# alipbcs/ZetaRay

Hardware: NVIDIA H100
Metric: Mpaths/s (1spp ReSTIR PT, 1080p) (higher is better)
Workload: dtype f32

## Files before the change

zetaray_b200/csrc/rdi.cu:

```cuda
#include "zr_pixel.cuh"
#include "zr_planes.h"
#include "zr_schedule.h"

#include "zr_rdi.cuh"

namespace zr
{
namespace
{
#ifndef ZR_RDI_TEMPORAL_THREADS
#define ZR_RDI_TEMPORAL_THREADS 768
#endif
#ifndef ZR_RDI_SPATIAL_THREADS
#define ZR_RDI_SPATIAL_THREADS 512
#endif
    static_assert(ZR_RDI_TEMPORAL_THREADS % 64 == 0 && ZR_RDI_SPATIAL_THREADS % 64 == 0, "a DI block is whole 8x8 groups");
    struct DiTemporalParked
    {
        Reservoir r;
        uint32_t pad[2];
    };
    static_assert(sizeof(DiTemporalParked) % 16 == 8, "DiTemporalParked must be 2 mod 4 words");
    constexpr size_t DI_TEMPORAL_SMEM_BYTES = (size_t)ZR_RDI_TEMPORAL_THREADS * sizeof(DiTemporalParked);

    template<uint32_t MF>
    __global__ void ZR_LB(ZR_RDI_TEMPORAL_THREADS) k_di_temporal(SceneDev sc, FrameView f, DIParams prm, zr_rdi_reservoir* __restrict__ resCurr,
        const zr_rdi_reservoir* __restrict__ resPrev, uint2* __restrict__ target, float4* __restrict__ finalImg, uint32_t dispX, uint32_t dispY,
        const uint32_t* __restrict__ order)
    {
        using SD = BSDF::ShadingDataT<MF>;
        extern __shared__ DiTemporalParked s_diTemporalParked[];
        const zr_frame_constants& fc = f.fc;
        uint2 sg = make_uint2(0, 0);
        const uint32_t groupFlat = order[blockIdx.x] * (ZR_RDI_TEMPORAL_THREADS / 64) + (threadIdx.x >> 6);
        const uint32_t tInGroup = threadIdx.x & 63;
        uint2 px = make_uint2(0xffffffffu, 0xffffffffu);
        if (groupFlat < dispX * dispY)
            px = SwizzleThreadGroup(groupFlat, 0, tInGroup & 7, tInGroup >> 3, 8, 8, dispX, 16, 4, 16 * dispY, sg);
        const long long t0 = clock64();
        bool act = !(px.x >= f.W || px.y >= f.H || px.y < prm.rowBegin || px.y >= prm.rowEnd);
        const uint32_t x = px.x, y = px.y;
        const size_t idx = act ? (size_t)y * f.W + x : 0;
        if (act)
        {
            const GFlags flags = FlagsAt(f.core, f.W, x, y);
            if (flags.invalid)
            {
                finalImg[idx] = f4(0, 0, 0, 0);
                act = false;
            }
            else if (flags.emissive && !prm.spatial)
            {
                WriteEmissive(fc, f, finalImg, idx);
                act = false;
            }
        }
        PixelT<SD> p;
        p.surface = SD::InitEmpty();
        p.pos = f3(0); p.normal = f3(0); p.roughness = 0;
        RNG rng_thread; rng_thread.State = 0;
        int numBsdfSamples = 0;
        if (act)
        {
            p = LoadPixel<SD>(f, sc, f.core, f.coat, x, y, false, x, y);
            rng_thread = RNG::Init(x, y, fc.FrameNum);
            numBsdfSamples = (!p.surface.GlossSpecular() && p.roughness < 0.3f) ? 2 : 1;
        }
        RNG rng_group = RNG::Init(groupFlat % dispX, groupFlat / dispX, fc.FrameNum);
        const uint32_t sampleSetIdx = rng_group.UniformUintBounded_Faster(sc.numSampleSets);
        Reservoir& r = s_diTemporalParked[threadIdx.x].r;
        RIS_InitialCandidates_Sync(r, act, sc, p.pos, p.normal, p.roughness, p.surface, sampleSetIdx, numBsdfSamples, rng_thread);
        if (prm.temporal)
        {
            float2 motionVec = f2(0, 0);
            TemporalCandidateT<SD> tc; tc.valid = false; tc.px = tc.py = 0; tc.pos = tc.normal = f3(0);
            tc.surface = SD::InitEmpty();
            ZR_PHASE();
            if (act)
            {
                motionVec = unpack_snorm16x2(__ldg(&f.me[idx].x));
                const float2 currUV = f2((float)x + 0.5f, (float)y + 0.5f) / f2((float)f.W, (float)f.H);
                const float2 prevUV = currUV - motionVec;
                tc = FindTemporalCandidate(f, sc, p.pos, p.normal, p.roughness, p.surface, prevUV);
            }
            TemporalResample1_Sync(act && tc.valid, sc, p.pos, p.normal, p.surface, tc, resPrev, f.W, r, rng_thread);
            if (act && prm.spatial)
            {
                const bool disoccluded = !tc.valid && (dot(motionVec, motionVec) > 0);
                r.target = disoccluded ? -r.target : r.target;
                WriteTarget(target, idx, r.target);
                r.target = Math::Sanitize(r.target);
            }
        }
        AccountCost(prm.costMap, f.W, f.H, px.x, px.y, t0);
        if (!act)
            return;
        if (prm.temporal || prm.reset)
        {
            zr_rdi_reservoir rec;
            r.Write(rec, prm.M_max);
            StoreRdi(&resCurr[idx], rec);
        }
        if (!prm.spatial || !prm.temporal)
            WriteFinal(fc, finalImg, idx, r.target * r.W);
    }

    template<uint32_t MF>
    __global__ void ZR_LB(ZR_RDI_SPATIAL_THREADS) k_di_spatial(SceneDev sc, FrameView f, DIParams prm, const zr_rdi_reservoir* __restrict__ resCurr,
        const uint2* __restrict__ target, float4* __restrict__ finalImg, uint32_t dispX, uint32_t dispY,
        const uint32_t* __restrict__ order)
    {
        using SD = BSDF::ShadingDataT<MF>;
        const zr_frame_constants& fc = f.fc;
        uint2 sg = make_uint2(0, 0);
        const uint32_t groupFlat = order[blockIdx.x] * (ZR_RDI_SPATIAL_THREADS / 64) + (threadIdx.x >> 6);
        const uint32_t tInGroup = threadIdx.x & 63;
        uint2 px = make_uint2(0xffffffffu, 0xffffffffu);
        if (groupFlat < dispX * dispY)
            px = SwizzleThreadGroup(groupFlat, 0, tInGroup & 7, tInGroup >> 3, 8, 8, dispX, 16, 4, 16 * dispY, sg);
        const long long t0 = clock64();
        bool active = px.x < f.W && px.y < f.H && px.y >= prm.rowBegin && px.y < prm.rowEnd;
        const int x = (int)px.x, y = (int)px.y;
        const size_t idx = active ? (size_t)y * f.W + x : 0;
        if (active)
        {
            const GFlags flags = FlagsAt(f.core, f.W, x, y);
            if (flags.invalid) active = false;
            else if (flags.emissive)
            {
                WriteEmissive(fc, f, finalImg, idx);
                active = false;
            }
        }
        PixelT<SD> p;
        p.surface = SD::InitEmpty();
        p.pos = f3(0); p.normal = f3(0); p.roughness = 0; p.z = 0;
        Reservoir r = Reservoir::Init();
        bool disoccluded = false;
        if (active)
        {
            p = LoadPixel<SD>(f, sc, f.core, f.coat, x, y, false, x, y);
            zr_rdi_reservoir rec;
            LoadRdi(&resCurr[idx], rec);
            r = Reservoir::Load(rec);
            if (r.lightIdx != UINT32_MAX_)
            {
                const zr_emissive_tri& tri = sc.emissives[r.lightIdx];
                r.lightID = tri.ID;
                const float3 vtx0 = Light::Vtx0(tri);
                const float3 vtx1 = Light::DecodeEmissiveTriV1(tri);
                const float3 vtx2 = Light::DecodeEmissiveTriV2(tri);
                r.lightPos = (1.0f - r.bary.x - r.bary.y) * vtx0 + r.bary.x * vtx1 + r.bary.y * vtx2;
                r.lightNormal = cross(vtx1 - vtx0, vtx2 - vtx0);
                r.lightNormal = dot(r.lightNormal, r.lightNormal) == 0 ? r.lightNormal : normalize(r.lightNormal);
                r.doubleSided = Light::IsDoubleSided(tri);
                r.target = LoadTarget(target, idx);
                disoccluded = r.target.x < 0 || r.target.y < 0 || r.target.z < 0;
                r.target = abs3(r.target);
            }
        }
        const uint32_t waveDisoccluded = __popc(__ballot_sync(0xffffffffu, active && disoccluded));
        RNG rng_group = RNG::Init(groupFlat % dispX, groupFlat / dispX, fc.FrameNum);
        rng_group.UniformUintBounded_Faster(sc.numSampleSets);
        const bool extra = !prm.stochasticSpatial || (rng_group.Uniform() < 0.6f);
        if (prm.extraDisocclusion)
            disoccluded = disoccluded && (waveDisoccluded > 3);
        int numSamples = extra ? 2 : 1;
        numSamples = !disoccluded ? numSamples : 4;
        RNG rng = RNG::Init((uint32_t)x, (uint32_t)y, fc.FrameNum);
        const float u0 = rng.Uniform();
        const int offset = (int)rng.UniformUintBounded_Faster(8);
        const float theta = u0 * TWO_PI;
        float sinTheta, cosTheta;
        zr_sincosf(theta, &sinTheta, &cosTheta);
        PairwiseMIS pairwiseMIS = PairwiseMIS::Init((uint32_t)numSamples, r);
        float3 samplePos[4]; int spx[4], spy[4]; uint32_t k = 0;
        ZR_PHASE();
        for (int i = 0; i < 4; i++)
        {
            if (!(active && i < numSamples)) continue;
            const float2 sampleUV = f2(c_disk32[((offset + i) & 31) * 2], c_disk32[((offset + i) & 31) * 2 + 1]);
            float2 rotated;
            rotated.x = dot(sampleUV, f2(cosTheta, -sinTheta));
            rotated.y = dot(sampleUV, f2(sinTheta, cosTheta));
            rotated = rotated * 16.0f;
            const float fx = fmaxf(rintf((float)x + rotated.x), 0.0f), fy = fmaxf(rintf((float)y + rotated.y), 0.0f);
            if (fx >= (float)f.W || fy >= (float)f.H) continue;
            const int qx = (int)fx, qy = (int)fy;
            float rough_i;
            const GFlags flags_i = FlagsAt(f.core, f.W, qx, qy, &rough_i);
            if (flags_i.invalid || flags_i.emissive) continue;
            const PixelT<SD> pi = LoadPixel<SD>(f, sc, f.core, f.coat, qx, qy, false, qx, qy);
            bool valid = PlaneHeuristicDI(pi.pos, p.normal, p.pos, p.z);
            valid = valid && (fabsf(rough_i - p.roughness) < 0.15f);
            if (!valid) continue;
            samplePos[k] = pi.pos; spx[k] = qx; spy[k] = qy;
            k++;
        }
        pairwiseMIS.k = k;
        for (uint32_t i = 0; i < 4; i++)
        {
            const bool go = active && (i < k);
            if (!__syncthreads_or(go))
                break;
            PixelT<SD> pi;
            pi.normal = f3(0);
            SD surface_i = SD::InitEmpty();
            Reservoir r_spatial = Reservoir::Init();
            float3 pos_i = f3(0);
            if (go)
            {
                pi = LoadPixel<SD>(f, sc, f.core, f.coat, spx[i], spy[i], false, spx[i], spy[i]);
                const uint4 c = ld128(&f.core[(size_t)spy[i] * f.W + spx[i]]);
                const float3 bc = f3((float)(c.z & 0xff) / 255.0f, (float)((c.z >> 8) & 0xff) / 255.0f, (float)((c.z >> 16) & 0xff) / 255.0f);
                const float bw = pi.flags.subsurface ? (float)(c.z >> 24) / 255.0f : 0.0f;
                pos_i = samplePos[i];
                const float3 wo_i = normalize(pi.origin - pos_i);
                surface_i = SD::Init(pi.normal, wo_i, pi.flags.metallic, pi.roughness, bc, BSDF::ETA_AIR,
                    pi.eta_next, pi.flags.transmissive, 0.0f, to_half(bw), pi.surface.coat_weight, pi.surface.coat_color,
                    pi.coatRoughness, pi.coatIor, sc.rho);
                zr_rdi_reservoir recN;
                LoadRdi(&resCurr[(size_t)spy[i] * f.W + spx[i]], recN);
                r_spatial = Reservoir::Load(recN);
            }
            pairwiseMIS.Stream_Sync(go, sc, r, p.pos, p.normal, p.surface, r_spatial, pos_i, pi.normal, surface_i, rng);
        }
        AccountCost(prm.costMap, f.W, f.H, px.x, px.y, t0);
        if (!active)
            return;
        pairwiseMIS.End(r, rng);
        const Reservoir rs = pairwiseMIS.r_s;
        WriteFinal(fc, finalImg, idx, rs.target * rs.W);
    }
}
}

struct zr_direct_pass
{
    uint32_t width = 0, height = 0;
    struct Sized
    {
        zr::Planes planes{ "zr_direct_pass" };
        zr_rdi_reservoir* d_res[2] = { nullptr, nullptr };
        uint2* d_target = nullptr;
        float4* d_final = nullptr;
    } sz;
    int currTemporalIdx = 0;
    bool isTemporalReservoirValid = false;
    bool resetTemporalTextures = true;
    bool patternLoaded = false;
    zr_direct_params params = Defaults();
    zr::LightingStrip strip{ "zr_direct_pass" };

    static zr_direct_params Defaults()
    {
        zr_direct_params p{};
        p.temporal_resample = 1; p.spatial_resample = 1; p.stochastic_spatial = 1; p.extra_disocclusion_sampling = 1;
        p.M_max = 20; p.alpha_min = 0.05f * 0.05f;
        return p;
    }
    zr_status Setup()
    {
        using zr::BSDF::MF_NONE; using zr::BSDF::MF_ALL;
        ZR_TRY(zr::ReserveParkedSmem(zr::k_di_temporal<MF_NONE>, ZR_RDI_TEMPORAL_THREADS, zr::DI_TEMPORAL_SMEM_BYTES, "zr_direct_pass: k_di_temporal"));
        ZR_TRY(zr::ReserveParkedSmem(zr::k_di_temporal<MF_ALL>, ZR_RDI_TEMPORAL_THREADS, zr::DI_TEMPORAL_SMEM_BYTES, "zr_direct_pass: k_di_temporal"));
        return ZR_OK;
    }
    zr_status OnWindowResized(uint32_t w, uint32_t h)
    {
        const size_t n = (size_t)w * h;
        Sized next;
        for (int i = 0; i < 2; i++) ZR_TRY(next.planes.Alloc(next.d_res[i], n));
        ZR_TRY(next.planes.Alloc(next.d_target, n));
        ZR_TRY(next.planes.Alloc(next.d_final, n));
        ZR_TRY(next.planes.Clear());
        sz = std::move(next);
        width = w; height = h;
        strip.ForgetSize();
        ResetFlags();
        return ZR_OK;
    }
    void ResetFlags() { currTemporalIdx = 0; isTemporalReservoirValid = false; resetTemporalTextures = true; }
    zr_status ResetTemporal()
    {
        ZR_TRY(sz.planes.Clear());
        ResetFlags();
        return ZR_OK;
    }
    zr_status LoadPattern()
    {
        if (patternLoaded) return ZR_OK;
        float pat[64];
        zr_status st = zr::read_asset("zr_direct_pass", "disk32.bin", pat, sizeof(pat));
        if (st != ZR_OK) return st;
        ZR_CUDA(cudaMemcpyToSymbol(zr::c_disk32, pat, 256));
        patternLoaded = true;
        return ZR_OK;
    }
    zr_status Render(const zr_frame_inputs* in, cudaStream_t stream)
    {
        using namespace zr;
        FrameView f;
        zr_status st = LightingFrame("zr_direct_pass", in, width, height, f);
        if (st != ZR_OK) return st;
        st = LoadPattern();
        if (st != ZR_OK) return st;
        const bool doTemporal = isTemporalReservoirValid && params.temporal_resample;
        const bool doSpatial = doTemporal && params.spatial_resample;
        if (doTemporal && (!in->prev.d_core || !in->prev.d_coat))
        {
            set_error("zr_direct_pass_render: temporal reuse needs the previous G-buffer");
            return ZR_ERR_INVALID_ARG;
        }
        DIParams prm{ doTemporal, doSpatial, params.stochastic_spatial, params.extra_disocclusion_sampling, params.M_max,
            params.alpha_min, resetTemporalTextures, strip.rowBegin, strip.ClampedRowEnd(height), strip.d_costMap };
        const uint32_t dispX = (width + 7) / 8, dispY = (height + 7) / 8;
        const int cur = currTemporalIdx;
        st = strip.Schedule(width, height, 8, 8, ZR_RDI_TEMPORAL_THREADS / 64, 0);
        if (st != ZR_OK) return st;
        st = strip.Schedule(width, height, 8, 8, ZR_RDI_SPATIAL_THREADS / 64, 1);
        if (st != ZR_OK) return st;
        const BlockSchedule& schedT = strip.sched[0];
        const BlockSchedule& schedS = strip.sched[1];
        const bool plain = (in->scene->materialFeatures & BSDF::MF_ALL) == 0;
        ZR_PROF("k_di_temporal", stream);
        (plain ? k_di_temporal<BSDF::MF_NONE> : k_di_temporal<BSDF::MF_ALL>)<<<schedT.count, ZR_RDI_TEMPORAL_THREADS, DI_TEMPORAL_SMEM_BYTES, stream>>>(in->scene->dev, f, prm, sz.d_res[cur], sz.d_res[1 - cur], sz.d_target, sz.d_final, dispX, dispY, schedT.d_order);
        ZR_LAUNCH_CHECK();
        strip.Exchange(sz.d_res[cur], width, height, 32u, stream);
        if (doSpatial)
        {
            ZR_PROF("k_di_spatial", stream);
            (plain ? k_di_spatial<BSDF::MF_NONE> : k_di_spatial<BSDF::MF_ALL>)<<<schedS.count, ZR_RDI_SPATIAL_THREADS, 0, stream>>>(in->scene->dev, f, prm, sz.d_res[cur], sz.d_target, sz.d_final, dispX, dispY, schedS.d_order);
            ZR_LAUNCH_CHECK();
        }
        isTemporalReservoirValid = true;
        currTemporalIdx = 1 - cur;
        resetTemporalTextures = false;
        return ZR_OK;
    }
};

extern "C"
{
    zr_status zr_direct_pass_create(uint32_t width, uint32_t height, zr_direct_pass** out) { return zr::CreatePass("zr_direct_pass", width, height, out); }
    zr_status zr_direct_pass_resize(zr_direct_pass* p, uint32_t width, uint32_t height) { return zr::ResizePass("zr_direct_pass", p, width, height); }
    zr_status zr_direct_pass_reset_temporal(zr_direct_pass* p) { return zr::ResetPass(p); }
    zr_status zr_direct_pass_default_params(zr_direct_params* out) { return zr::DefaultParams<zr_direct_pass>(out); }
    zr_status zr_direct_pass_set_params(zr_direct_pass* p, const zr_direct_params* params)
    {
        if (!p || !params) return ZR_ERR_INVALID_ARG;
        if (params->M_max == 0 || params->M_max > 31) { zr::set_error("zr_direct_pass_set_params: M_max must be in 1..31 (5-bit field)"); return ZR_ERR_INVALID_ARG; }
        p->params = *params;
        return ZR_OK;
    }
    zr_status zr_direct_pass_render(zr_direct_pass* p, const zr_frame_inputs* in, void* stream)
    {
        if (!p) return ZR_ERR_INVALID_ARG;
        return p->Render(in, (cudaStream_t)stream);
    }
    zr_status zr_direct_pass_set_rows(zr_direct_pass* p, uint32_t y0, uint32_t y1) { return p ? p->strip.SetRows(y0, y1, p->height) : ZR_ERR_INVALID_ARG; }
    zr_status zr_direct_pass_set_halo_exchange(zr_direct_pass* p, zr_halo_exchange_fn fn, void* user) { return p ? p->strip.SetHaloExchange(fn, user) : ZR_ERR_INVALID_ARG; }
    zr_status zr_direct_pass_set_schedule_costs(zr_direct_pass* p, const double* h_tile_cost, uint32_t tiles_x, uint32_t tiles_y)
    {
        return p ? p->strip.SetScheduleCosts(h_tile_cost, tiles_x, tiles_y, p->width, p->height) : ZR_ERR_INVALID_ARG;
    }
    zr_status zr_direct_pass_set_cost_map(zr_direct_pass* p, void* d_cycles) { return p ? p->strip.SetCostMap(d_cycles) : ZR_ERR_INVALID_ARG; }
    zr_status zr_direct_pass_get_output(zr_direct_pass* p, zr_direct_output id, zr_image2d* out)
    {
        if (!p || !out) return ZR_ERR_INVALID_ARG;
        const uint32_t w = p->width, h = p->height;
        switch (id)
        {
        case ZR_DIRECT_FINAL: *out = zr_image2d{ p->sz.d_final, w, h, w * 16u, 16u }; break;
        case ZR_DIRECT_RESERVOIR_CURR: *out = zr_image2d{ p->sz.d_res[1 - p->currTemporalIdx], w, h, w * 32u, 32u }; break;
        case ZR_DIRECT_TARGET: *out = zr_image2d{ p->sz.d_target, w, h, w * 8u, 8u }; break;
        default: zr::set_error("zr_direct_pass_get_output: unknown output id"); return ZR_ERR_INVALID_ARG;
        }
        return ZR_OK;
    }
    zr_status zr_direct_pass_describe_io(zr_direct_pass* p, zr_resource_use* uses, int* n)
    {
        if (!p || !uses || !n) return ZR_ERR_INVALID_ARG;
        uses[0] = zr_resource_use{ ZR_RES_GBUFFER_CURR, 0 };
        uses[1] = zr_resource_use{ ZR_RES_GBUFFER_PREV, 0 };
        uses[2] = zr_resource_use{ ZR_RES_SCENE_BVH, 0 };
        uses[3] = zr_resource_use{ ZR_RES_ALIAS_TABLE, 0 };
        uses[4] = zr_resource_use{ ZR_RES_DI_FINAL, 1 };
        *n = 5;
        return ZR_OK;
    }
    void zr_direct_pass_destroy(zr_direct_pass* p) { delete p; }
}
```

zetaray_b200/csrc/renderer.cu:

```cuda
#include <cuda_runtime.h>
#include <vector>
#include "../../include/zr_abi.h"
#include "zr_common.cuh"

struct zr_renderer
{
    uint32_t width = 0, height = 0;
    zr_scene* scene = nullptr;
    zr_gbuffer gbuffer[2]{};
    int curr = 0;
    uint64_t framesRendered = 0;
    zr_gbuffer_pass* gbufferPass = nullptr;
    zr_direct_pass* direct = nullptr;
    zr_indirect_pass* indirect = nullptr;
    zr_gi_pass* gi = nullptr;
    zr_integrator integrator = ZR_INTEGRATOR_RESTIR_PT;
    zr_compositing_pass* compositing = nullptr;
    zr_taa_pass* taa = nullptr;
    zr_svgf_pass* svgf = nullptr;
    zr_auto_exposure_pass* ae = nullptr;
    zr_display_pass* display = nullptr;
    cudaStream_t side = nullptr;
    cudaEvent_t evGBuffer = nullptr, evDirect = nullptr;
    bool twoStreams = true;
    zr_comm* comm = nullptr;
    int rank = 0, world = 1;
    std::vector<uint32_t> bounds;
    bool gatherOutput = true;
    static constexpr uint32_t HALO = 32;
    struct HookCtx { zr_renderer* r; int whichComm; } hookMain{ this, 0 }, hookSide{ this, 1 };
    zr_status hookStatus = ZR_OK;
    static void HaloHook(void* user, const zr_image2d* planes, int n, void* stream)
    {
        HookCtx* h = (HookCtx*)user;
        zr_renderer* r = h->r;
        const int which = (r->twoStreams && stream == (void*)r->side) ? 1 : 0;
        const zr_status s = zr_comm_exchange_halos(r->comm, which, r->bounds.data(), HALO, planes, n, stream);
        if (s != ZR_OK) r->hookStatus = s;
    }
    static void ReduceHook(void* user, uint32_t* d_values, uint32_t n, void* stream)
    {
        zr_renderer* r = (zr_renderer*)user;
        const zr_status s = zr_comm_allreduce_u32(r->comm, 0, d_values, n, stream);
        if (s != ZR_OK) r->hookStatus = s;
    }

    zr_status ApplyShard()
    {
        const bool sharded = comm && world > 1;
        const uint32_t y0 = sharded ? bounds[rank] : 0, y1 = sharded ? bounds[rank + 1] : height;
        zr_halo_exchange_fn hook = sharded ? HaloHook : nullptr;
        zr_status s = zr_gbuffer_pass_set_rows(gbufferPass, y0 > HALO ? y0 - HALO : 0, y1 + HALO < height ? y1 + HALO : height);
        if (s == ZR_OK) s = zr_direct_pass_set_rows(direct, y0, y1);
        if (s == ZR_OK) s = zr_indirect_pass_set_rows(indirect, y0, y1);
        if (s == ZR_OK) s = zr_compositing_pass_set_rows(compositing, y0 > 0 ? y0 - 1 : 0, y1 + 1 < height ? y1 + 1 : height);
        if (s == ZR_OK) s = zr_taa_pass_set_rows(taa, y0, y1);
        if (s == ZR_OK) s = zr_direct_pass_set_halo_exchange(direct, hook, &hookSide);
        if (s == ZR_OK) s = zr_indirect_pass_set_halo_exchange(indirect, hook, &hookMain);
        if (s == ZR_OK && gi) s = zr_gi_pass_set_rows(gi, y0, y1);
        if (s == ZR_OK && gi) s = zr_gi_pass_set_halo_exchange(gi, hook, &hookMain);
        if (s == ZR_OK && svgf) s = zr_svgf_pass_set_rows(svgf, y0, y1);
        if (s == ZR_OK && svgf) s = zr_svgf_pass_set_halo_exchange(svgf, hook, &hookMain);
        if (s == ZR_OK && ae) s = zr_auto_exposure_pass_set_rows(ae, y0, y1);
        if (s == ZR_OK && ae) s = zr_auto_exposure_pass_set_reduce(ae, sharded ? ReduceHook : nullptr, this);
        if (s == ZR_OK && display) s = zr_display_pass_set_rows(display, y0, y1);
        return s;
    }
    zr_status TakeHookStatus()
    {
        const zr_status s = hookStatus;
        hookStatus = ZR_OK;
        return s;
    }
    void ReleaseDisplay()
    {
        if (ae) zr_auto_exposure_pass_destroy(ae);
        if (display) zr_display_pass_destroy(display);
        ae = nullptr; display = nullptr;
    }

    void Release()
    {
        if (gbufferPass) zr_gbuffer_pass_destroy(gbufferPass);
        if (direct) zr_direct_pass_destroy(direct);
        if (indirect) zr_indirect_pass_destroy(indirect);
        if (gi) zr_gi_pass_destroy(gi);
        gi = nullptr;
        if (compositing) zr_compositing_pass_destroy(compositing);
        if (taa) zr_taa_pass_destroy(taa);
        if (svgf) zr_svgf_pass_destroy(svgf);
        svgf = nullptr;
        ReleaseDisplay();
        gbufferPass = nullptr; direct = nullptr; indirect = nullptr; compositing = nullptr; taa = nullptr;
        for (int i = 0; i < 2; i++) zr_gbuffer_free(&gbuffer[i]);
        if (side) cudaStreamDestroy(side);
        if (evGBuffer) cudaEventDestroy(evGBuffer);
        if (evDirect) cudaEventDestroy(evDirect);
        side = nullptr; evGBuffer = evDirect = nullptr;
    }
};

extern "C"
{
    zr_status zr_renderer_create(const zr_renderer_desc* desc, zr_scene* scene, zr_renderer** out)
    {
        if (!desc || !scene || !out || !desc->width || !desc->height)
        {
            zr::set_error("zr_renderer_create: bad args");
            return ZR_ERR_INVALID_ARG;
        }
        zr_renderer* r = new zr_renderer();
        r->width = desc->width; r->height = desc->height; r->scene = scene; r->twoStreams = desc->two_streams != 0;
        zr_status s = ZR_OK;
        for (int i = 0; i < 2 && s == ZR_OK; i++) s = zr_gbuffer_alloc(desc->width, desc->height, desc->with_tridiff, &r->gbuffer[i]);
        if (s == ZR_OK) s = zr_gbuffer_pass_create(&r->gbufferPass);
        if (s == ZR_OK) s = zr_direct_pass_create(desc->width, desc->height, &r->direct);
        if (s == ZR_OK) s = zr_indirect_pass_create(desc->width, desc->height, &r->indirect);
        if (s == ZR_OK) s = zr_compositing_pass_create(desc->width, desc->height, &r->compositing);
        if (s == ZR_OK) s = zr_taa_pass_create(desc->width, desc->height, &r->taa);
        if (s == ZR_OK && cudaStreamCreateWithFlags(&r->side, cudaStreamNonBlocking) != cudaSuccess) s = ZR_ERR_CUDA;
        if (s == ZR_OK && cudaEventCreateWithFlags(&r->evGBuffer, cudaEventDisableTiming) != cudaSuccess) s = ZR_ERR_CUDA;
        if (s == ZR_OK && cudaEventCreateWithFlags(&r->evDirect, cudaEventDisableTiming) != cudaSuccess) s = ZR_ERR_CUDA;
        if (s != ZR_OK) { r->Release(); delete r; return s; }
        *out = r;
        return ZR_OK;
    }

    void zr_renderer_destroy(zr_renderer* r)
    {
        if (!r) return;
        r->Release();
        delete r;
    }

    zr_status zr_renderer_render(zr_renderer* r, const zr_frame_constants* fc, void* stream_)
    {
        if (!r || !fc) return ZR_ERR_INVALID_ARG;
        if (fc->RenderWidth != r->width || fc->RenderHeight != r->height)
        {
            zr::set_error("zr_renderer_render: frame is %ux%u but the renderer was sized %ux%u", fc->RenderWidth, fc->RenderHeight,
                r->width, r->height);
            return ZR_ERR_INVALID_ARG;
        }
        cudaStream_t stream = (cudaStream_t)stream_;
        zr_status s;
        if (r->framesRendered == 0)
        {
            s = zr_prelighting_render(r->scene, stream);
            if (s != ZR_OK) return s;
        }
        s = zr_presample_emissives(r->scene, fc->FrameNum, stream);
        if (s != ZR_OK) return s;
        s = zr_build_light_voxel_grid(r->scene, fc, stream);
        if (s != ZR_OK) return s;

        r->curr ^= 1;
        zr_frame_inputs in;
        in.frame = *fc;
        in.curr = r->gbuffer[r->curr];
        in.prev = r->gbuffer[r->curr ^ 1];
        in.scene = r->scene;

        s = zr_gbuffer_pass_render(r->gbufferPass, &in, stream);
        if (s != ZR_OK) return s;
        cudaStream_t directStream = stream;
        if (r->twoStreams)
        {
            ZR_CUDA(cudaEventRecord(r->evGBuffer, stream));
            ZR_CUDA(cudaStreamWaitEvent(r->side, r->evGBuffer, 0));
            directStream = r->side;
        }
        s = zr_direct_pass_render(r->direct, &in, directStream);
        if (s != ZR_OK) return s;
        s = r->integrator != ZR_INTEGRATOR_RESTIR_PT ? zr_gi_pass_render(r->gi, &in, stream) : zr_indirect_pass_render(r->indirect, &in, stream);
        if (s != ZR_OK) return s;
        if (r->twoStreams)
        {
            ZR_CUDA(cudaEventRecord(r->evDirect, r->side));
            ZR_CUDA(cudaStreamWaitEvent(stream, r->evDirect, 0));
        }
        s = r->TakeHookStatus();
        if (s != ZR_OK) return s;
        zr_image2d di, ind, comp;
        s = zr_direct_pass_get_output(r->direct, ZR_DIRECT_FINAL, &di);
        if (s != ZR_OK) return s;
        s = r->integrator != ZR_INTEGRATOR_RESTIR_PT ? zr_gi_pass_get_output(r->gi, ZR_GI_FINAL, &ind)
                                                     : zr_indirect_pass_get_output(r->indirect, ZR_INDIRECT_FINAL, &ind);
        if (s != ZR_OK) return s;
        if (r->comm && r->world > 1)
        {
            zr_image2d planes[3] = { di, ind, zr_image2d{} };
            s = zr_taa_pass_get_output(r->taa, &planes[2]);
            if (s != ZR_OK) return s;
            s = zr_comm_exchange_halos(r->comm, 0, r->bounds.data(), zr_renderer::HALO, planes, 3, stream);
            if (s != ZR_OK) return s;
        }
        s = zr_compositing_pass_render(r->compositing, &in, di.d_ptr, ind.d_ptr, stream);
        if (s != ZR_OK) return s;
        s = zr_compositing_pass_get_output(r->compositing, &comp);
        if (s != ZR_OK) return s;
        if (r->svgf)
        {
            s = zr_svgf_pass_render(r->svgf, &in, comp.d_ptr, stream);
            if (s != ZR_OK) return s;
            s = r->TakeHookStatus();
            if (s != ZR_OK) return s;
            s = zr_svgf_pass_get_output(r->svgf, ZR_SVGF_DENOISED, &comp);
            if (s != ZR_OK) return s;
        }
        zr_image2d exposure{};
        if (r->ae)
        {
            s = zr_auto_exposure_pass_render(r->ae, &in, comp.d_ptr, stream);
            if (s != ZR_OK) return s;
            s = r->TakeHookStatus();
            if (s != ZR_OK) return s;
            s = zr_auto_exposure_pass_get_output(r->ae, &exposure);
            if (s != ZR_OK) return s;
        }
        s = zr_taa_pass_render(r->taa, &in, comp.d_ptr, stream);
        if (s != ZR_OK) return s;
        zr_image2d img;
        s = zr_taa_pass_get_output(r->taa, &img);
        if (s != ZR_OK) return s;
        zr_image2d shown{};
        if (r->display)
        {
            s = zr_display_pass_render(r->display, &in, img.d_ptr, exposure.d_ptr, stream);
            if (s != ZR_OK) return s;
            s = zr_display_pass_get_output(r->display, &shown);
            if (s != ZR_OK) return s;
        }
        if (r->comm && r->world > 1 && r->gatherOutput)
        {
            s = zr_comm_gather_rows(r->comm, r->bounds.data(), &img, 0, stream);
            if (s != ZR_OK) return s;
            if (r->display) s = zr_comm_gather_rows(r->comm, r->bounds.data(), &shown, 0, stream);
            if (s != ZR_OK) return s;
        }
        r->framesRendered++;
        return ZR_OK;
    }

    zr_status zr_renderer_set_integrator(zr_renderer* r, zr_integrator method)
    {
        if (!r) return ZR_ERR_INVALID_ARG;
        if (method != ZR_INTEGRATOR_PATH_TRACING && method != ZR_INTEGRATOR_RESTIR_GI && method != ZR_INTEGRATOR_RESTIR_PT)
        {
            zr::set_error("zr_renderer_set_integrator: unknown integrator %d (path tracing = 0, ReSTIR GI = 1, ReSTIR PT = 2)", (int)method);
            return ZR_ERR_INVALID_ARG;
        }
        if (method == r->integrator) return ZR_OK;
        zr_status s = ZR_OK;
        if (method != ZR_INTEGRATOR_RESTIR_PT)
        {
            if (!r->gi) s = zr_gi_pass_create(r->width, r->height, &r->gi);
            else s = zr_gi_pass_reset_temporal(r->gi);
            if (s == ZR_OK) s = zr_gi_pass_set_method(r->gi, method);
            if (s == ZR_OK) s = r->ApplyShard();
        }
        else
            s = zr_indirect_pass_reset_temporal(r->indirect);
        if (s != ZR_OK) return s;
        r->integrator = method;
        return ZR_OK;
    }
    zr_status zr_renderer_set_denoiser(zr_renderer* r, int enable, zr_svgf_pass** out_pass)
    {
        if (!r) return ZR_ERR_INVALID_ARG;
        zr_status s = ZR_OK;
        if (enable && !r->svgf)
        {
            s = zr_svgf_pass_create(r->width, r->height, &r->svgf);
            if (s == ZR_OK) s = r->ApplyShard();
            if (s != ZR_OK && r->svgf) { zr_svgf_pass_destroy(r->svgf); r->svgf = nullptr; }
        }
        if (!enable && r->svgf) { zr_svgf_pass_destroy(r->svgf); r->svgf = nullptr; }
        if (out_pass) *out_pass = r->svgf;
        return s;
    }
    zr_status zr_renderer_set_display(zr_renderer* r, int enable, zr_auto_exposure_pass** out_ae, zr_display_pass** out_display)
    {
        if (!r) return ZR_ERR_INVALID_ARG;
        zr_status s = ZR_OK;
        if (enable && !r->ae)
        {
            s = zr_auto_exposure_pass_create(r->width, r->height, &r->ae);
            if (s == ZR_OK) s = zr_display_pass_create(r->width, r->height, &r->display);
            if (s == ZR_OK) s = r->ApplyShard();
            if (s != ZR_OK) r->ReleaseDisplay();
        }
        if (!enable) r->ReleaseDisplay();
        if (out_ae) *out_ae = r->ae;
        if (out_display) *out_display = r->display;
        return s;
    }
    zr_status zr_renderer_get_display_output(zr_renderer* r, zr_image2d* out)
    {
        if (!r || !out) return ZR_ERR_INVALID_ARG;
        if (!r->display) { zr::set_error("zr_renderer_get_display_output: the display stage is off (zr_renderer_set_display)"); return ZR_ERR_NOT_INITIALIZED; }
        return zr_display_pass_get_output(r->display, out);
    }
    zr_status zr_renderer_set_shard(zr_renderer* r, zr_comm* comm, const uint32_t* bounds, int gather_output)
    {
        if (!r) return ZR_ERR_INVALID_ARG;
        if (!comm)
        {
            r->comm = nullptr; r->world = 1; r->rank = 0; r->bounds.clear();
            return r->ApplyShard();
        }
        if (!bounds) { zr::set_error("zr_renderer_set_shard: bounds missing"); return ZR_ERR_INVALID_ARG; }
        int rank = 0, world = 1;
        zr_status s = zr_comm_rank(comm, &rank, &world);
        if (s != ZR_OK) return s;
        if (bounds[0] != 0 || bounds[world] != r->height) { zr::set_error("zr_renderer_set_shard: bounds must cover [0, height)"); return ZR_ERR_INVALID_ARG; }
        for (int q = 0; q < world; q++)
            if (bounds[q + 1] <= bounds[q] || (q + 1 < world && bounds[q + 1] % 32 != 0))
            {
                zr::set_error("zr_renderer_set_shard: strip bounds must increase and be multiples of 32 rows");
                return ZR_ERR_INVALID_ARG;
            }
        r->comm = comm; r->rank = rank; r->world = world; r->gatherOutput = gather_output != 0;
        r->bounds.assign(bounds, bounds + world + 1);
        return r->ApplyShard();
    }
    zr_status zr_renderer_get_gi_pass(zr_renderer* r, zr_gi_pass** gi)
    {
        if (!r || !gi) return ZR_ERR_INVALID_ARG;
        *gi = r->gi;
        return ZR_OK;
    }
    zr_status zr_renderer_apply_scene_settings(zr_renderer* r, int use_lvg, uint32_t out_applied[2])
    {
        if (!r) return ZR_ERR_INVALID_ARG;
        const zr_alias_entry* table = nullptr; uint32_t numEmissive = 0;
        zr_status s = zr_scene_get_alias_table(r->scene, &table, &numEmissive);
        if (s != ZR_OK) return s;
        constexpr uint32_t MIN_NUM_LIGHTS_PRESAMPLING = (uint32_t)((0.5 * 1024 * 1024) / sizeof(zr_presampled_tri));
        static_assert(MIN_NUM_LIGHTS_PRESAMPLING == 13107, "sizeof(PresampledEmissiveTriangle) must be 40");
        const bool presampling = numEmissive >= MIN_NUM_LIGHTS_PRESAMPLING;
        const bool lvg = use_lvg && presampling;
        s = presampling ? zr_scene_set_presampling(r->scene, 128, 512) : zr_scene_set_presampling(r->scene, 0, 0);
        if (s != ZR_OK) return s;
        const uint32_t dim[3] = { 32, 8, 40 }, none[3] = { 0, 0, 0 };
        const float ext[3] = { 0.6f, 0.45f, 0.6f };
        s = zr_scene_set_light_voxel_grid(r->scene, lvg ? dim : none, ext, 0.1f);
        if (s != ZR_OK) return s;
        if (out_applied) { out_applied[0] = presampling; out_applied[1] = lvg; }
        return ZR_OK;
    }

    zr_status zr_renderer_get_output(zr_renderer* r, zr_image2d* out)
    {
        if (!r || !out) return ZR_ERR_INVALID_ARG;
        return zr_taa_pass_get_output(r->taa, out);
    }
    zr_status zr_renderer_get_passes(zr_renderer* r, zr_gbuffer_pass** g, zr_direct_pass** d, zr_indirect_pass** i,
        zr_compositing_pass** c, zr_taa_pass** t)
    {
        if (!r) return ZR_ERR_INVALID_ARG;
        if (g) *g = r->gbufferPass;
        if (d) *d = r->direct;
        if (i) *i = r->indirect;
        if (c) *c = r->compositing;
        if (t) *t = r->taa;
        return ZR_OK;
    }
    zr_status zr_renderer_get_gbuffer(zr_renderer* r, int previous, zr_gbuffer* out)
    {
        if (!r || !out) return ZR_ERR_INVALID_ARG;
        *out = r->gbuffer[previous ? r->curr ^ 1 : r->curr];
        return ZR_OK;
    }
}
```

zetaray_b200/csrc/rpt_spatial.cu:

```cuda
#include "zr_rpt_spatial.h"
#include "zr_rpt_shift.cuh"
#include "zr_tma.cuh"

namespace zr
{
namespace
{
    using namespace RPT;

    __global__ void __launch_bounds__(256) k_spatial_classify(FrameView f, RptParams prm, const zr_rpt_reservoir* __restrict__ resIn,
        const uint16_t* __restrict__ neighbor, uint32_t* __restrict__ queue, uint32_t* __restrict__ counters, uint32_t capacity)
    {
        __shared__ uint32_t s_count[SpatialQueued::NUM_CLASSES], s_base[SpatialQueued::NUM_CLASSES];
        const uint32_t x = blockIdx.x * 32 + (threadIdx.x & 31);
        const uint32_t y = prm.rowBegin + blockIdx.y * 8 + (threadIdx.x >> 5);
        if (threadIdx.x < SpatialQueued::NUM_CLASSES) s_count[threadIdx.x] = 0;
        __syncthreads();
        uint32_t cls[2] = { NO_ITEM, NO_ITEM };
        if (x < f.W && y < f.H && y < prm.rowEnd)
        {
            const GFlags flags = FlagsAt(f.core, f.W, (int)x, (int)y);
            int nx = 0, ny = 0;
            if (!(flags.invalid || flags.emissive) && NeighborOf(f, neighbor, (int)x, (int)y, nx, ny))
            {
                const uint4 q0 = ld128(&resIn[(size_t)y * f.W + x]);
                const uint4 qn = ld128(&resIn[(size_t)ny * f.W + nx]);
                const bool selfEmpty = (q0.x & 0xf) == Reconnection::EMPTY, nEmpty = (qn.x & 0xf) == Reconnection::EMPTY;
                const uint32_t M_n = (qn.x >> 4) & 0xf;
                if (asfloat(q0.y) != 0 && !selfEmpty && M_n > 0) cls[0] = ShiftClass(q0.x);
                if (!nEmpty) cls[1] = ShiftClass(qn.x);
            }
        }
        const uint32_t item[2] = { x | (y << 16), x | (y << 16) | (1u << 31) };
        AppendItems(cls, item, queue, counters, capacity, s_count, s_base);
    }

    struct MergeSmem
    {
        uint4 rec[2][1024][4];
        float val[2][1024];
        float sum[2][1024];
        uint8_t cls[1024];
        uint8_t visited[1024];
        unsigned long long bar[2];
    };

    __global__ void __launch_bounds__(1024, 1) k_spatial_merge(const CUtensorMap* __restrict__ pMapIn, FrameView f, RptParams prm,
        const zr_rpt_reservoir* __restrict__ resIn, zr_rpt_reservoir* __restrict__ resOut, const float4* __restrict__ target,
        float4* __restrict__ finalImg, const uint16_t* __restrict__ neighbor, const uint16_t* __restrict__ threadMap,
        const ShiftResult* __restrict__ shiftRes, uint32_t tilesX, uint32_t tileRow0, uint32_t numTiles, uint32_t swizzled)
    {
        extern __shared__ __align__(1024) unsigned char smemRaw[];
        MergeSmem& sm = *reinterpret_cast<MergeSmem*>(smemRaw);
        const zr_frame_constants& fc = f.fc;
        const uint32_t t = threadIdx.x, lane = t & 31, warp = t >> 5;
        constexpr uint32_t TILE_BYTES = 1024 * 64;

        if (t == 0)
        {
            tma::MbarInit(reinterpret_cast<uint64_t*>(&sm.bar[0]), 1);
            tma::MbarInit(reinterpret_cast<uint64_t*>(&sm.bar[1]), 1);
            tma::FenceBarrierInit();
        }
        __syncthreads();
        auto issue = [&](uint32_t tile, uint32_t stage)
        {
            const uint32_t tx = tile % tilesX, ty = tileRow0 + tile / tilesX;
            uint64_t* bar = reinterpret_cast<uint64_t*>(&sm.bar[stage]);
            tma::MbarArriveExpectTx(bar, TILE_BYTES);
            if (swizzled) tma::Load3D(&sm.rec[stage][0][0], pMapIn, bar, 0, (int32_t)(tx * 16), (int32_t)(ty * 32));
            else tma::Load2D(&sm.rec[stage][0][0], pMapIn, bar, (int32_t)(tx * 32 * 8), (int32_t)(ty * 32));
        };
        if (t == 0 && blockIdx.x < numTiles)
            issue(blockIdx.x, 0);

        uint32_t pfFlags = 0xff, pfNb = 0xffff, pfMap = 0x8000;
        float4 pfTg = f4(0, 0, 0, 0);
        auto prefetch = [&](uint32_t tile)
        {
            const uint32_t tX = tile % tilesX, tY = tileRow0 + tile / tilesX;
            const uint32_t px = tX * 32 + lane, py = tY * 32 + warp;
            pfFlags = 0xff; pfNb = 0xffff; pfMap = 0x8000;
            if (px < f.W && py < f.H && py >= prm.rowBegin && py < prm.rowEnd)
            {
                const size_t i = (size_t)py * f.W + px;
                pfFlags = __ldg(&f.core[i].w) & 0xff;
                pfNb = __ldg(&neighbor[i]);
                pfTg = __ldg(&target[i]);
            }
            const uint32_t sx = tX * 32 + (warp & 3) * 8 + (lane & 7), sy = tY * 32 + (warp >> 2) * 4 + (lane >> 3);
            if (sx < f.W && sy < f.H)
                pfMap = prm.sortSpatial ? __ldg(&threadMap[(size_t)sy * f.W + sx]) : (31u | (31u << 7));
        };
        if (blockIdx.x < numTiles)
            prefetch(blockIdx.x);

        uint32_t it = 0;
        for (uint32_t tile = blockIdx.x; tile < numTiles; tile += gridDim.x, it++)
        {
            const uint32_t stage = it & 1, parity = (it >> 1) & 1;
            const uint32_t tileX = tile % tilesX, tileY = tileRow0 + tile / tilesX;
            if (t == 0 && tile + gridDim.x < numTiles)
            {
                tma::FenceProxyAsync();
                issue(tile + gridDim.x, stage ^ 1);
            }
            const int x = (int)(tileX * 32 + lane), y = (int)(tileY * 32 + warp);
            const bool inImage = (uint32_t)x < f.W && (uint32_t)y < f.H;
            const size_t idx = inImage ? (size_t)y * f.W + x : 0;
            bool act = false;
            {
                const GFlags flags = DecodeFlags(pfFlags);
                act = !(flags.invalid || flags.emissive);
            }
            int nx = 0, ny = 0;
            bool hasN = false;
            const float4 tg = pfTg;
            const uint32_t mapEnc = pfMap;
            uint4 sh0 = make_uint4(0, 0, 0, 0);
            float2 sh1 = f2(0, 0);
            uint4 n0 = make_uint4(Reconnection::EMPTY, 0, 0, 0), n1 = make_uint4(0, 0, 0, 0);
            if (act)
            {
                const uint32_t ox = pfNb & 0xff, oy = pfNb >> 8;
                hasN = ox != 0xff;
                nx = (int)ox - 32 + x; ny = (int)oy - 32 + y;
                if (hasN)
                {
                    const uint4* nrec = reinterpret_cast<const uint4*>(&resIn[(size_t)ny * f.W + nx]);
                    n0 = __ldg(&nrec[0]); n1 = __ldg(&nrec[1]);
                    asm volatile("prefetch.global.L1 [%0];" :: "l"(nrec + 2));
                    const uint4* sp = reinterpret_cast<const uint4*>(&shiftRes[idx]);
                    sh0 = __ldg(&sp[0]);
                    sh1 = __ldg(reinterpret_cast<const float2*>(&sp[1]));
                }
            }
            if (tile + gridDim.x < numTiles)
                prefetch(tile + gridDim.x);
            sm.visited[t] = 0;
            tma::MbarWait(reinterpret_cast<uint64_t*>(&sm.bar[stage]), parity);

            zr_rpt_reservoir rec;
            {
                const uint4* line = &sm.rec[stage][t & ~1u][0];
                const uint32_t c0 = (t & 1u) * 4u, sw = swizzled ? ((t >> 1) & 7u) : 0u;
                uint4 v[4] = { line[(c0 + 0) ^ sw], line[(c0 + 1) ^ sw], line[(c0 + 2) ^ sw], line[(c0 + 3) ^ sw] };
                memcpy(&rec, v, 64);
            }
            Reservoir r_curr = Reservoir::Load_NonReconnection(rec);
            r_curr.target = f3(tg.x, tg.y, tg.z);
            const float wsum0 = act ? r_curr.w_sum : 0.0f;
            uint32_t M_max = prm.M_max_spatial;
            M_max = !r_curr.rc.Empty() && r_curr.rc.lobe_k_min_1 == BSDF::GLOSSY_T ? (M_max < 4 ? M_max : 4) : M_max;
            uint32_t cls = 0, M_new = 0;
            bool changed = false, surfKMin1Tr = false;
            zr_rpt_reservoir recN;
            Reservoir r_spatial = Reservoir::Init();
            if (act && !hasN)
                cls = 1;
            else if (act)
            {
                memset(&recN, 0, sizeof(recN));
                memcpy(&recN, &n0, 16); memcpy(reinterpret_cast<unsigned char*>(&recN) + 16, &n1, 16);
                r_spatial = Reservoir::Load_NonReconnection(recN);
                if ((r_curr.w_sum != 0) && !r_curr.rc.Empty() && (r_spatial.M > 0))
                {
                    const float target_spatial = sh1.x;
                    if (target_spatial > 0)
                    {
                        const float selfJ = (r_curr.rc.IsCase3() && r_curr.rc.lobe_k_min_1 == BSDF::ALL) ? 1.0f : asfloat(rec.jacobian_or_seed_nee);
                        const float targetLum_curr = r_curr.W > 0 ? r_curr.w_sum / r_curr.W : 0;
                        const float jacobian = selfJ > 0 ? sh1.y / selfJ : 0;
                        const float numerator = (float)r_curr.M * targetLum_curr;
                        const float denom = numerator + (float)r_spatial.M * target_spatial * jacobian;
                        const float m_curr = denom > 0 ? numerator / denom : 0;
                        r_curr.w_sum *= m_curr;
                    }
                }
                M_new = r_curr.M + r_spatial.M;
                if (r_spatial.rc.Empty())
                    cls = 2;
                else
                {
                    cls = 3;
                    M_max = r_spatial.rc.x_k_in_motion ? (M_max < 4 ? M_max : 4) : M_max;
                    r_spatial.rc.x_k_in_motion = false;
                    const float nJ = (r_spatial.rc.IsCase3() && r_spatial.rc.lobe_k_min_1 == BSDF::ALL) ? 1.0f : asfloat(recN.jacobian_or_seed_nee);
                    const float3 shTarget = f3(asfloat(sh0.x), asfloat(sh0.y), asfloat(sh0.z));
                    const float shJ = fabsf(asfloat(sh0.w));
                    surfKMin1Tr = (sh0.w >> 31) != 0;
                    const float targetLum_curr = Math::Luminance(shTarget);
                    const float targetLum_spatial = r_spatial.W > 0 ? r_spatial.w_sum / r_spatial.W : 0;
                    const float jacobian = nJ > 0 ? shJ / nJ : 0;
                    if (targetLum_curr > 1e-6f && jacobian > 1e-5f && jacobian < 100)
                    {
                        const uint3 h = RNG::PCG3d(make_uint3((uint32_t)x, (uint32_t)y, (uint32_t)y));
                        RNG rng = RNG::Init(h.x, h.z, fc.FrameNum + 511);
                        const float numerator = (float)r_spatial.M * targetLum_spatial;
                        const float denom = numerator / jacobian + (float)r_curr.M * targetLum_curr;
                        const float m_spatial = denom > 0 ? numerator / denom : 0;
                        const float w_spatial = m_spatial * r_spatial.W * targetLum_curr;
                        if (r_curr.Update(w_spatial, shTarget, r_spatial.rc, rng))
                        {
                            const uint4* nrec = reinterpret_cast<const uint4*>(&resIn[(size_t)ny * f.W + nx]);
                            const uint4 n2 = __ldg(&nrec[2]), n3 = __ldg(&nrec[3]);
                            memcpy(reinterpret_cast<unsigned char*>(&recN) + 32, &n2, 16);
                            memcpy(reinterpret_cast<unsigned char*>(&recN) + 48, &n3, 16);
                            r_spatial.Load_Reconnection(recN);
                            r_curr.rc = r_spatial.rc;
                            r_curr.rc.partialJacobian = shJ;
                            changed = true;
                        }
                    }
                    const float targetLum = Math::Luminance(r_curr.target);
                    r_curr.W = targetLum > 0 ? r_curr.w_sum / targetLum : 0;
                    r_curr.M = M_new;
                }
            }
            sm.val[0][t] = wsum0;
            sm.val[1][t] = act ? r_curr.w_sum : 0.0f;
            sm.cls[t] = (uint8_t)cls;
            __syncthreads();

            {
                const int sx = (int)(tileX * 32 + (warp & 3) * 8 + (lane & 7)), sy = (int)(tileY * 32 + (warp >> 2) * 4 + (lane >> 3));
                bool on = (uint32_t)sx < f.W && (uint32_t)sy < f.H;
                int lx = sx - (int)(tileX * 32), ly = sy - (int)(tileY * 32);
                if (mapEnc & (1u << 15)) on = false;
                lx += (int)(mapEnc & 0x3f) - 31;
                ly += (int)((mapEnc >> 7) & 0x3f) - 31;
                if (on && ((uint32_t)lx >= 32u || (uint32_t)ly >= 32u)) on = false;
                const uint32_t lp = on ? (uint32_t)(ly * 32 + lx) : 0;
                const float v0 = on ? sm.val[0][lp] : 0.0f, v1 = on ? sm.val[1][lp] : 0.0f;
                const uint32_t c = on ? sm.cls[lp] : 0;
                const float waveSum = WaveSum32(v0);
                float waveAcc = WaveSum32(c == 1 ? v1 : 0.0f);
                waveAcc += WaveSum32(c == 2 ? v1 : 0.0f);
                const float total = waveAcc + WaveSum32(c == 3 ? v1 : 0.0f);
                if (on)
                {
                    sm.sum[0][lp] = waveSum; sm.sum[1][lp] = total;
                    sm.visited[lp] = 1;
                }
            }
            __syncthreads();

            if (act && sm.visited[t])
            {
                const float avgEx0 = (sm.sum[0][t] - wsum0) / 32.0f;
                if (cls == 1)
                {
                    if (prm.boilingSuppression) SuppressOutlier(avgEx0, r_curr);
                    WriteOutputColor(fc, finalImg, idx, r_curr.target * r_curr.W);
                    CopyToNextFrame(rec, &resOut[idx], r_curr, M_max);
                }
                else if (cls == 2)
                {
                    if (prm.boilingSuppression) SuppressOutlier(avgEx0, r_curr);
                    const float targetLum = Math::Luminance(r_curr.target);
                    r_curr.W = targetLum > 0 ? r_curr.w_sum / targetLum : 0;
                    r_curr.M = M_new;
                    CopyToNextFrame(rec, &resOut[idx], r_curr, M_max);
                    WriteOutputColor(fc, finalImg, idx, r_curr.target * r_curr.W);
                }
                else
                {
                    if (prm.boilingSuppression)
                        SuppressOutlier((sm.sum[1][t] - r_curr.w_sum) / 32.0f, r_curr);
                    if (changed)
                    {
                        const uint32_t mmax = surfKMin1Tr ? (M_max < 4 ? M_max : 4) : M_max;
                        zr_rpt_reservoir out;
                        r_curr.Write(out, mmax);
                        StoreRecord(&resOut[idx], out);
                    }
                    else
                        CopyToNextFrame(rec, &resOut[idx], r_curr, M_max);
                    WriteOutputColor(fc, finalImg, idx, r_curr.target * r_curr.W);
                }
            }
            __syncthreads();
        }
    }
}

zr_status ShiftStreams::Init()
{
    int dev = 0;
    ZR_CUDA(cudaGetDevice(&dev));
    ZR_CUDA(cudaDeviceGetAttribute(&numSMs, cudaDevAttrMultiProcessorCount, dev));
    ZR_CUDA(cudaFuncSetAttribute(k_spatial_merge, cudaFuncAttributeMaxDynamicSharedMemorySize, (int)sizeof(MergeSmem)));
    ZR_TRY(SetupShifts<false>());
    ZR_TRY(SetupTemporalShifts());
    for (int i = 0; i < 2; i++)
    {
        ZR_CUDA(cudaStreamCreateWithFlags(&aux[i], cudaStreamNonBlocking));
        ZR_CUDA(cudaEventCreateWithFlags(&evJoin[i], cudaEventDisableTiming));
    }
    ZR_CUDA(cudaEventCreateWithFlags(&evFork, cudaEventDisableTiming));
    return ZR_OK;
}

ShiftStreams::~ShiftStreams()
{
    for (int i = 0; i < 2; i++)
    {
        if (aux[i]) cudaStreamDestroy(aux[i]);
        if (evJoin[i]) cudaEventDestroy(evJoin[i]);
    }
    if (evFork) cudaEventDestroy(evFork);
}

zr_status SpatialQueued::Build(uint32_t w, uint32_t h, const zr_rpt_reservoir* res0, const zr_rpt_reservoir* res1)
{
    width = w; height = h;
    const size_t n = (size_t)w * h;
    capacity = 2 * n;
    ZR_TRY(planes.Alloc(d_queue, NUM_CLASSES * capacity, false));
    ZR_TRY(planes.Alloc(d_counters, 16, false));
    ZR_TRY(planes.Alloc(d_shift, n));
    ZR_TRY(planes.Alloc(d_flags, n));
    ZR_TRY(planes.Alloc(d_maps, 2, false));
    const zr_rpt_reservoir* res[2] = { res0, res1 };
    CUtensorMap maps[2];
    swizzled = (w % 2) == 0;
    for (int i = 0; i < 2; i++)
    {
        mapBase[i] = res[i];
        bool ok;
        if (swizzled)
        {
            const uint64_t dims[3] = { 16, w / 2, h };
            const uint64_t strides[2] = { 128, (uint64_t)w * 64 };
            const uint32_t box[3] = { 16, 16, 32 };
            ok = tma::EncodeWords(&maps[i], res[i], 3, dims, strides, box, true);
        }
        else
            ok = tma::EncodePlane2D(&maps[i], res[i], w, h, 64, (uint64_t)w * 64, 32, 32);
        if (!ok)
        {
            set_error("zr_indirect_pass: cuTensorMapEncodeTiled failed for the %ux%u reservoir plane", w, h);
            return ZR_ERR_CUDA;
        }
    }
    ZR_CUDA(cudaMemcpy(d_maps, maps, sizeof(maps), cudaMemcpyHostToDevice));
    return planes.Clear();
}

zr_status SpatialQueued::Run(const ShiftStreams& ss, const SceneDev& sc, const FrameView& f, const RptParams& prm, const zr_rpt_reservoir* resIn,
    zr_rpt_reservoir* resOut, const float4* target, float4* finalImg, const uint16_t* neighbor, const uint16_t* threadMap, bool plain, cudaStream_t stream)
{
    const int plane = resIn == mapBase[0] ? 0 : (resIn == mapBase[1] ? 1 : -1);
    if (plane < 0) { set_error("zr_indirect_pass: spatial input is not one of the pass's reservoir planes"); return ZR_ERR_INVALID_ARG; }
    const uint32_t rows = prm.rowEnd - prm.rowBegin;
    ZR_CUDA(cudaMemsetAsync(d_counters, 0, 16 * sizeof(uint32_t), stream));
    {
        ZR_PROF("k_spatial_classify", stream);
        k_spatial_classify<<<dim3((width + 31) / 32, (rows + 7) / 8), 256, 0, stream>>>(f, prm, resIn, neighbor, d_queue, d_counters, (uint32_t)capacity);
        ZR_LAUNCH_CHECK();
    }
    {
        ZR_PROF("k_shift", stream);
        const zr_status ls = LaunchShifts<false>(*this, ss, sc, f, prm, resIn, nullptr, neighbor, plain, stream);
        zr::prof_after();
        if (ls != ZR_OK) return ls;
        cudaError_t e = cudaGetLastError();
        if (e != cudaSuccess) return zr::cuda_fail(e, "k_shift launch");
    }
    {
        const uint32_t tilesX = (width + 31) / 32;
        const uint32_t tileRow0 = prm.rowBegin / 32, tileRow1 = (prm.rowEnd + 31) / 32;
        const uint32_t numTiles = tilesX * (tileRow1 - tileRow0);
        const uint32_t grid = numTiles < (uint32_t)ss.numSMs ? numTiles : (uint32_t)ss.numSMs;
        ZR_PROF("k_spatial_merge", stream);
        k_spatial_merge<<<grid, 1024, sizeof(MergeSmem), stream>>>(d_maps + plane, f, prm, resIn, resOut, target, finalImg, neighbor, threadMap,
            d_shift, tilesX, tileRow0, numTiles, swizzled ? 1u : 0u);
        ZR_LAUNCH_CHECK();
    }
    return ZR_OK;
}
}
```

Measured before the change: 323.6.

## Run indirect chain on high-priority stream, direct DI on low-priority side stream

Moves the G-buffer and indirect (ReSTIR PT) passes onto a new high-priority 'chain' stream, with the direct-lighting pass on a low-priority side stream that waits only on the G-buffer. The indirect pass is issued before direct so the critical path starts first. The RPT spatial aux streams get high priority too. DI kernels get half-size blocks with explicit min-blocks launch bounds derived from register budgets, which lets several blocks share an SM and trades register headroom for occupancy. The register caps risk spills.

```diff
diff --git a/zetaray_b200/csrc/rdi.cu b/zetaray_b200/csrc/rdi.cu
--- a/zetaray_b200/csrc/rdi.cu
+++ b/zetaray_b200/csrc/rdi.cu
@@ -9,12 +9,15 @@
 namespace
 {
 #ifndef ZR_RDI_TEMPORAL_THREADS
-#define ZR_RDI_TEMPORAL_THREADS 768
+#define ZR_RDI_TEMPORAL_THREADS 384
 #endif
 #ifndef ZR_RDI_SPATIAL_THREADS
-#define ZR_RDI_SPATIAL_THREADS 512
+#define ZR_RDI_SPATIAL_THREADS 256
 #endif
     static_assert(ZR_RDI_TEMPORAL_THREADS % 64 == 0 && ZR_RDI_SPATIAL_THREADS % 64 == 0, "a DI block is whole 8x8 groups");
+    constexpr int DI_TEMPORAL_REGS = 80, DI_SPATIAL_REGS = 128;
+    static_assert(ZR_RDI_TEMPORAL_THREADS * DI_TEMPORAL_REGS <= 65536 && ZR_RDI_SPATIAL_THREADS * DI_SPATIAL_REGS <= 65536,
+        "a DI block must fit the register file at its bound");
     struct DiTemporalParked
     {
         Reservoir r;
@@ -24,7 +27,7 @@
     constexpr size_t DI_TEMPORAL_SMEM_BYTES = (size_t)ZR_RDI_TEMPORAL_THREADS * sizeof(DiTemporalParked);
 
     template<uint32_t MF>
-    __global__ void ZR_LB(ZR_RDI_TEMPORAL_THREADS) k_di_temporal(SceneDev sc, FrameView f, DIParams prm, zr_rdi_reservoir* __restrict__ resCurr,
+    __global__ void __launch_bounds__(ZR_RDI_TEMPORAL_THREADS, 65536 / (ZR_RDI_TEMPORAL_THREADS * DI_TEMPORAL_REGS)) k_di_temporal(SceneDev sc, FrameView f, DIParams prm, zr_rdi_reservoir* __restrict__ resCurr,
         const zr_rdi_reservoir* __restrict__ resPrev, uint2* __restrict__ target, float4* __restrict__ finalImg, uint32_t dispX, uint32_t dispY,
         const uint32_t* __restrict__ order)
     {
@@ -106,7 +109,7 @@
     }
 
     template<uint32_t MF>
-    __global__ void ZR_LB(ZR_RDI_SPATIAL_THREADS) k_di_spatial(SceneDev sc, FrameView f, DIParams prm, const zr_rdi_reservoir* __restrict__ resCurr,
+    __global__ void __launch_bounds__(ZR_RDI_SPATIAL_THREADS, 65536 / (ZR_RDI_SPATIAL_THREADS * DI_SPATIAL_REGS)) k_di_spatial(SceneDev sc, FrameView f, DIParams prm, const zr_rdi_reservoir* __restrict__ resCurr,
         const uint2* __restrict__ target, float4* __restrict__ finalImg, uint32_t dispX, uint32_t dispY,
         const uint32_t* __restrict__ order)
     {
diff --git a/zetaray_b200/csrc/renderer.cu b/zetaray_b200/csrc/renderer.cu
--- a/zetaray_b200/csrc/renderer.cu
+++ b/zetaray_b200/csrc/renderer.cu
@@ -20,8 +20,9 @@
     zr_svgf_pass* svgf = nullptr;
     zr_auto_exposure_pass* ae = nullptr;
     zr_display_pass* display = nullptr;
+    cudaStream_t chain = nullptr;
     cudaStream_t side = nullptr;
-    cudaEvent_t evGBuffer = nullptr, evDirect = nullptr;
+    cudaEvent_t evFork = nullptr, evGBuffer = nullptr, evChain = nullptr, evDirect = nullptr;
     bool twoStreams = true;
     zr_comm* comm = nullptr;
     int rank = 0, world = 1;
@@ -93,10 +94,11 @@
         ReleaseDisplay();
         gbufferPass = nullptr; direct = nullptr; indirect = nullptr; compositing = nullptr; taa = nullptr;
         for (int i = 0; i < 2; i++) zr_gbuffer_free(&gbuffer[i]);
+        if (chain) cudaStreamDestroy(chain);
         if (side) cudaStreamDestroy(side);
-        if (evGBuffer) cudaEventDestroy(evGBuffer);
-        if (evDirect) cudaEventDestroy(evDirect);
-        side = nullptr; evGBuffer = evDirect = nullptr;
+        for (cudaEvent_t e : { evFork, evGBuffer, evChain, evDirect })
+            if (e) cudaEventDestroy(e);
+        chain = side = nullptr; evFork = evGBuffer = evChain = evDirect = nullptr;
     }
 };
 
@@ -118,9 +120,12 @@
         if (s == ZR_OK) s = zr_indirect_pass_create(desc->width, desc->height, &r->indirect);
         if (s == ZR_OK) s = zr_compositing_pass_create(desc->width, desc->height, &r->compositing);
         if (s == ZR_OK) s = zr_taa_pass_create(desc->width, desc->height, &r->taa);
-        if (s == ZR_OK && cudaStreamCreateWithFlags(&r->side, cudaStreamNonBlocking) != cudaSuccess) s = ZR_ERR_CUDA;
-        if (s == ZR_OK && cudaEventCreateWithFlags(&r->evGBuffer, cudaEventDisableTiming) != cudaSuccess) s = ZR_ERR_CUDA;
-        if (s == ZR_OK && cudaEventCreateWithFlags(&r->evDirect, cudaEventDisableTiming) != cudaSuccess) s = ZR_ERR_CUDA;
+        int leastPriority = 0, greatestPriority = 0;
+        if (s == ZR_OK && cudaDeviceGetStreamPriorityRange(&leastPriority, &greatestPriority) != cudaSuccess) s = ZR_ERR_CUDA;
+        if (s == ZR_OK && cudaStreamCreateWithPriority(&r->chain, cudaStreamNonBlocking, greatestPriority) != cudaSuccess) s = ZR_ERR_CUDA;
+        if (s == ZR_OK && cudaStreamCreateWithPriority(&r->side, cudaStreamNonBlocking, leastPriority) != cudaSuccess) s = ZR_ERR_CUDA;
+        for (cudaEvent_t* e : { &r->evFork, &r->evGBuffer, &r->evChain, &r->evDirect })
+            if (s == ZR_OK && cudaEventCreateWithFlags(e, cudaEventDisableTiming) != cudaSuccess) s = ZR_ERR_CUDA;
         if (s != ZR_OK) { r->Release(); delete r; return s; }
         *out = r;
         return ZR_OK;
@@ -161,22 +166,31 @@
         in.prev = r->gbuffer[r->curr ^ 1];
         in.scene = r->scene;
 
-        s = zr_gbuffer_pass_render(r->gbufferPass, &in, stream);
-        if (s != ZR_OK) return s;
-        cudaStream_t directStream = stream;
+        cudaStream_t chainStream = stream, directStream = stream;
         if (r->twoStreams)
         {
-            ZR_CUDA(cudaEventRecord(r->evGBuffer, stream));
+            ZR_CUDA(cudaEventRecord(r->evFork, stream));
+            ZR_CUDA(cudaStreamWaitEvent(r->chain, r->evFork, 0));
+            chainStream = r->chain;
+            directStream = r->side;
+        }
+        s = zr_gbuffer_pass_render(r->gbufferPass, &in, chainStream);
+        if (s != ZR_OK) return s;
+        if (r->twoStreams)
+        {
+            ZR_CUDA(cudaEventRecord(r->evGBuffer, chainStream));
             ZR_CUDA(cudaStreamWaitEvent(r->side, r->evGBuffer, 0));
-            directStream = r->side;
-        }
+        }
+        s = r->integrator != ZR_INTEGRATOR_RESTIR_PT ? zr_gi_pass_render(r->gi, &in, chainStream)
+                                                     : zr_indirect_pass_render(r->indirect, &in, chainStream);
+        if (s != ZR_OK) return s;
         s = zr_direct_pass_render(r->direct, &in, directStream);
         if (s != ZR_OK) return s;
-        s = r->integrator != ZR_INTEGRATOR_RESTIR_PT ? zr_gi_pass_render(r->gi, &in, stream) : zr_indirect_pass_render(r->indirect, &in, stream);
-        if (s != ZR_OK) return s;
         if (r->twoStreams)
         {
-            ZR_CUDA(cudaEventRecord(r->evDirect, r->side));
+            ZR_CUDA(cudaEventRecord(r->evChain, chainStream));
+            ZR_CUDA(cudaEventRecord(r->evDirect, directStream));
+            ZR_CUDA(cudaStreamWaitEvent(stream, r->evChain, 0));
             ZR_CUDA(cudaStreamWaitEvent(stream, r->evDirect, 0));
         }
         s = r->TakeHookStatus();
diff --git a/zetaray_b200/csrc/rpt_spatial.cu b/zetaray_b200/csrc/rpt_spatial.cu
--- a/zetaray_b200/csrc/rpt_spatial.cu
+++ b/zetaray_b200/csrc/rpt_spatial.cu
@@ -292,9 +292,11 @@
     ZR_CUDA(cudaFuncSetAttribute(k_spatial_merge, cudaFuncAttributeMaxDynamicSharedMemorySize, (int)sizeof(MergeSmem)));
     ZR_TRY(SetupShifts<false>());
     ZR_TRY(SetupTemporalShifts());
+    int leastPriority = 0, greatestPriority = 0;
+    ZR_CUDA(cudaDeviceGetStreamPriorityRange(&leastPriority, &greatestPriority));
     for (int i = 0; i < 2; i++)
     {
-        ZR_CUDA(cudaStreamCreateWithFlags(&aux[i], cudaStreamNonBlocking));
+        ZR_CUDA(cudaStreamCreateWithPriority(&aux[i], cudaStreamNonBlocking, greatestPriority));
         ZR_CUDA(cudaEventCreateWithFlags(&evJoin[i], cudaEventDisableTiming));
     }
     ZR_CUDA(cudaEventCreateWithFlags(&evFork, cudaEventDisableTiming));
```

Result: faster. 334.1, median of 6 (+3.2%).
